# pyannote/pyannote-video

Hardware: AMD Instinct MI355X
Metric: frames/sec end-to-end detect->embed->cluster, 1080p@25fps (higher is better)
Workload: dtype f32 (detector scores, embedder) / f64 (tracker, clustering) / u8 frames; an f16 screening pass with a proven error bound decides which windows the detector's exact f32 chain is evaluated for -- results identical to dense f32 scoring (`dense_scoring`)

## Files before the change

pyannote-video_amd/csrc/api.hip:

```cpp
#include "pvf_internal.h"
#include <algorithm>
#include <cmath>
#include <cstdlib>
#include <string>
#include <thread>

#define API_BEGIN try {
#define API_END                                                        \
    return 0;                                                          \
    }                                                                  \
    catch (const std::exception& e) { pvf_set_error(e.what()); return -1; } \
    catch (...) { pvf_set_error("unknown error"); return -2; }

#define ENTER(c, h)                                                \
    Ctx* c = pvf_ctx(h);                                           \
    std::lock_guard<std::recursive_mutex> _api_lock(c->api_mu);    \
    HIP_CHECK(hipSetDevice(c->device))
#define ENTER_DET(c, h)                                            \
    Ctx* c = pvf_ctx(h);                                           \
    std::lock_guard<std::recursive_mutex> _det_lock(c->det_mu);    \
    HIP_CHECK(hipSetDevice(c->device))
#define ENTER_BOTH(c, h)                                           \
    Ctx* c = pvf_ctx(h);                                           \
    std::lock_guard<std::recursive_mutex> _det_lock(c->det_mu);    \
// ... 618 lines not shown
    for (int i = 0; i < n; ++i) f[i] = c->frame(frames[i]);
    ert_run(c, f, boxes, n, pts);
    API_END
}

extern "C" int32_t pvf_debug_landmarks_shape(pvf_handle h, const pvf_handle* frames, const pvf_rect_i32* boxes, int32_t n, int32_t* pts, float* shape)
{
    API_BEGIN
    ENTER(c, h);
    PVF_REQUIRE(n >= 0 && ((frames && boxes && pts && shape) || n == 0), "pvf_debug_landmarks_shape: bad arguments");
    if (n == 0) return 0;
    std::vector<Frame> f(n);
    for (int i = 0; i < n; ++i) f[i] = c->frame(frames[i]);
    ert_run(c, f, boxes, n, pts, shape);
    API_END
}

static uint8_t* make_face_chips(Ctx* c, const pvf_handle* frames, const int32_t* pts, int n)
{
    const EmbedModel& e = c->emb;
    PVF_REQUIRE(e.loaded, "embedder not loaded");
    std::vector<ChipJob> jobs(n);
    for (int i = 0; i < n; ++i) {
        ChipDetails d;
        face_chip_details(e, pts + (size_t)i * 68 * 2, &d);
        jobs[i] = chip_plan(c->frame(frames[i]), d);
    }
    const size_t bytes = (size_t)n * e.chip_size * e.chip_size * 3;
    c->s_trk0.ensure(bytes);
    chip_extract_batch(c, jobs, c->s_trk0.as<uint8_t>());
    return c->s_trk0.as<uint8_t>();
}

extern "C" int32_t pvf_face_chips(pvf_handle h, const pvf_handle* frames, const int32_t* pts, int32_t n, uint8_t* chips)
{
    API_BEGIN
    ENTER(c, h);
    if (n == 0) return 0;
    uint8_t* d = make_face_chips(c, frames, pts, n);
    HIP_CHECK(hipMemcpyAsync(chips, d, (size_t)n * 150 * 150 * 3, hipMemcpyDeviceToHost, c->stream));
    HIP_CHECK(hipStreamSynchronize(c->stream));
    API_END
}

extern "C" int32_t pvf_embed(pvf_handle h, const pvf_handle* frames, const int32_t* pts, int32_t n, float* out)
{
    API_BEGIN
    ENTER(c, h);
    if (n == 0) return 0;
    const int CH = 4096;
    for (int i0 = 0; i0 < n; i0 += CH) {
        const int m = std::min(CH, n - i0);
        uint8_t* d = make_face_chips(c, frames + i0, pts + (size_t)i0 * 136, m);
        resnet_forward(c, d, m, out + (size_t)i0 * 128);
    }
    API_END
}

extern "C" int32_t pvf_landmarks_embed(pvf_handle h, const pvf_handle* frames, const pvf_rect_i32* boxes, int32_t n, int32_t* pts, float* out)
{
    API_BEGIN
    ENTER(c, h);
    PVF_REQUIRE(n >= 0, "pvf_landmarks_embed: bad arguments");
    if (n == 0) return 0;
    PVF_REQUIRE(frames && boxes && pts && out, "pvf_landmarks_embed: bad arguments");
    {
        std::vector<Frame> f(n);
        for (int i = 0; i < n; ++i) f[i] = c->frame(frames[i]);
        ert_run(c, f, boxes, n, pts);
    }
    const int CH = 4096;
    for (int i0 = 0; i0 < n; i0 += CH) {
        const int m = std::min(CH, n - i0);
        uint8_t* d = make_face_chips(c, frames + i0, pts + (size_t)i0 * 136, m);
        resnet_forward(c, d, m, out + (size_t)i0 * 128);
    }
    API_END
}

extern "C" int32_t pvf_embed_chips(pvf_handle h, const uint8_t* chips, int32_t n, float* out)
{
    API_BEGIN
    ENTER(c, h);
    if (n == 0) return 0;
    const size_t bytes = (size_t)n * 150 * 150 * 3;
    c->s_trk0.ensure(bytes);
    HIP_CHECK(hipMemcpyAsync(c->s_trk0.p, chips, bytes, hipMemcpyHostToDevice, c->stream));
    resnet_forward(c, c->s_trk0.as<uint8_t>(), n, out);
    API_END
}

extern "C" int32_t pvf_jitter_plan(int32_t J, uint64_t seed, double* out)
{
    API_BEGIN
    jitter_check_count("pvf_jitter_plan", J);
    PVF_REQUIRE(out || J == 0, "pvf_jitter_plan: bad arguments");
    jitter_plan_rows(J, seed, out);
    API_END
}

static int32_t debug_jitter_chips(const char* who, pvf_handle h, const uint8_t* chips, int32_t n, int32_t J, uint64_t seed, uint8_t* out, bool via_transform)
{
    API_BEGIN
    ENTER(c, h);
    jitter_check_count(who, J);
    PVF_REQUIRE(n >= 0 && J >= 1 && ((chips && (out || via_transform)) || n == 0), std::string(who) + ": bad arguments");
    if (n == 0) return 0;
// ... 20 lines not shown
}

static int32_t jitter_entry_check(const char* who, int32_t n, int32_t J, bool pointers)
{
    API_BEGIN
    jitter_check_count(who, J);
    PVF_REQUIRE(n >= 0 && (pointers || n == 0), std::string(who) + ": bad arguments");
    API_END
}

extern "C" int32_t pvf_embed_jitter(pvf_handle h, const pvf_handle* frames, const int32_t* pts, int32_t n, int32_t J, uint64_t seed, float* out)
{
    if (jitter_entry_check("pvf_embed_jitter", n, J, frames && pts && out)) return -1;
    if (J <= 1) return pvf_embed(h, frames, pts, n, out);
    API_BEGIN
    ENTER(c, h);
    const int CH = 4096;
    for (int i0 = 0; i0 < n; i0 += CH) {
        const int m = std::min(CH, n - i0);
        uint8_t* d = make_face_chips(c, frames + i0, pts + (size_t)i0 * 136, m);
        jitter_embed_dev(c, d, m, J, seed, out + (size_t)i0 * 128);
    }
    API_END
}

extern "C" int32_t pvf_landmarks_embed_jitter(pvf_handle h, const pvf_handle* frames, const pvf_rect_i32* boxes, int32_t n, int32_t J, uint64_t seed,
                                              int32_t* pts, float* out)
{
    if (jitter_entry_check("pvf_landmarks_embed_jitter", n, J, frames && boxes && pts && out)) return -1;
    if (J <= 1) return pvf_landmarks_embed(h, frames, boxes, n, pts, out);
    API_BEGIN
    ENTER(c, h);
    if (n == 0) return 0;
    {
        std::vector<Frame> f(n);
        for (int i = 0; i < n; ++i) f[i] = c->frame(frames[i]);
        ert_run(c, f, boxes, n, pts);
    }
    const int CH = 4096;
    for (int i0 = 0; i0 < n; i0 += CH) {
        const int m = std::min(CH, n - i0);
        uint8_t* d = make_face_chips(c, frames + i0, pts + (size_t)i0 * 136, m);
        jitter_embed_dev(c, d, m, J, seed, out + (size_t)i0 * 128);
    }
    API_END
}

extern "C" int32_t pvf_embed_chips_jitter(pvf_handle h, const uint8_t* chips, int32_t n, int32_t J, uint64_t seed, float* out)
{
    if (jitter_entry_check("pvf_embed_chips_jitter", n, J, chips && out)) return -1;
    if (J <= 1) return pvf_embed_chips(h, chips, n, out);
    API_BEGIN
    ENTER(c, h);
    if (n == 0) return 0;
    const size_t bytes = (size_t)n * 150 * 150 * 3;
    c->s_trk0.ensure(bytes);
    HIP_CHECK(hipMemcpyAsync(c->s_trk0.p, chips, bytes, hipMemcpyHostToDevice, c->stream));
    jitter_embed_dev(c, c->s_trk0.as<uint8_t>(), n, J, seed, out);
    API_END
}

extern "C" int32_t pvf_debug_extract_chip(pvf_handle h, pvf_handle frame, const double rect[4], double cs, double sn, int32_t rows,
                                          int32_t cols, uint8_t* out)
{
    API_BEGIN
    ENTER(c, h);
    ChipDetails d{rect[0], rect[1], rect[2], rect[3], cs, sn, rows, cols};
    std::vector<ChipJob> jobs{chip_plan(c->frame(frame), d)};
    const size_t bytes = (size_t)rows * cols * 3;
    c->s_trk0.ensure(bytes);
    chip_extract_batch(c, jobs, c->s_trk0.as<uint8_t>());
    HIP_CHECK(hipMemcpyAsync(out, c->s_trk0.p, bytes, hipMemcpyDeviceToHost, c->stream));
    HIP_CHECK(hipStreamSynchronize(c->stream));
    API_END
}
// ... 415 lines not shown
```

pyannote-video_amd/csrc/chip.hip:

```cpp
#include "pvf_internal.h"
#include <algorithm>
#include <cmath>

static void pyr_down2_dims(int ih, int iw, int* oh, int* ow)
{
    if (ih <= 8 || iw <= 8) { *oh = 0; *ow = 0; return; }
    *oh = (ih - 3) / 2; *ow = (iw - 3) / 2;
}

ChipJob chip_plan(const Frame& f, const ChipDetails& d) { return chip_plan_geom(f.d, f.h, f.w, d); }

struct DevPyrJob { const uint8_t* src; int stride_w, x0, y0; uint8_t* dst; int dh, dw; };

#define PD_TW 32
#define PD_TH 8
__global__ void __launch_bounds__(256) pyr_down2_k(const DevPyrJob* __restrict__ jobs)
{
    __shared__ uint16_t hs[2 * PD_TH + 3][PD_TW][4];
    const DevPyrJob j = jobs[blockIdx.z];
    const int c0 = blockIdx.x * PD_TW, r0 = blockIdx.y * PD_TH;
    if (j.dst == nullptr || r0 >= j.dh || c0 >= j.dw) return;
    const int tid = threadIdx.x;
    const int rows_in = min(2 * PD_TH + 3, 2 * (j.dh - r0) + 3);
    for (int idx = tid; idx < (2 * PD_TH + 3) * PD_TW; idx += 256) {
        const int sr = idx / PD_TW, oc = idx % PD_TW;
        if (sr >= rows_in || c0 + oc >= j.dw) continue;
        const uint8_t* p = j.src + ((size_t)(j.y0 + 2 * r0 + sr) * j.stride_w + (j.x0 + 2 * (c0 + oc))) * 3;
        const uint32_t d0 = *reinterpret_cast<const uint32_t*>(p), d1 = *reinterpret_cast<const uint32_t*>(p + 4);
        const uint32_t d2 = *reinterpret_cast<const uint32_t*>(p + 8), d3 = *reinterpret_cast<const uint32_t*>(p + 11);
        const uint32_t h0 = (d0 & 0xffu) + 4 * (d0 >> 24) + 6 * ((d1 >> 16) & 0xffu) + 4 * ((d2 >> 8) & 0xffu) + ((d3 >> 8) & 0xffu);
        const uint32_t h1 = ((d0 >> 8) & 0xffu) + 4 * (d1 & 0xffu) + 6 * (d1 >> 24) + 4 * ((d2 >> 16) & 0xffu) + ((d3 >> 16) & 0xffu);
        const uint32_t h2 = ((d0 >> 16) & 0xffu) + 4 * ((d1 >> 8) & 0xffu) + 6 * (d2 & 0xffu) + 4 * (d2 >> 24) + (d3 >> 24);
        *reinterpret_cast<uint2*>(&hs[sr][oc][0]) = make_uint2(h0 | (h1 << 16), h2);
    }
    __syncthreads();
    const int c = c0 + (tid & (PD_TW - 1)), rl = tid >> 5, r = r0 + rl;
    if (r >= j.dh || c >= j.dw) return;
    const int oc = tid & (PD_TW - 1);
    uint32_t acc[3];
#pragma unroll
    for (int k = 0; k < 3; ++k)
        acc[k] = hs[2 * rl][oc][k] + 4u * hs[2 * rl + 1][oc][k] + 6u * hs[2 * rl + 2][oc][k] + 4u * hs[2 * rl + 3][oc][k] + hs[2 * rl + 4][oc][k];
    uint8_t* o = j.dst + ((size_t)r * j.dw + c) * 3;
    o[0] = (uint8_t)(acc[0] / 256); o[1] = (uint8_t)(acc[1] / 256); o[2] = (uint8_t)(acc[2] / 256);
}

__global__ void __launch_bounds__(256) transform_k(const DevXfJob* __restrict__ jobs, uint8_t* __restrict__ out, int rows, int cols)
{
    const DevXfJob j = jobs[blockIdx.z];
    const int c = blockIdx.x * blockDim.x + threadIdx.x;
    const int r = blockIdx.y;
    if (c >= cols) return;
    uint8_t* o = out + ((size_t)blockIdx.z * rows * cols + (size_t)r * cols + c) * 3;
    if (j.src == nullptr) { o[0] = 0; o[1] = 0; o[2] = 0; return; }
    const double px = j.m[0] * c + j.m[1] * r + j.b[0];
    const double py = j.m[2] * c + j.m[3] * r + j.b[1];
    const double fx = floor(px), fy = floor(py);
    if (!(fx >= 0 && fy >= 0 && fx + 1 < j.sw && fy + 1 < j.sh)) { o[0] = 0; o[1] = 0; o[2] = 0; return; }
    const int left = (int)fx, top = (int)fy;
    const double lr = px - left, tb = py - top;
    const uint8_t* ptl = j.src + ((size_t)(j.y0 + top) * j.stride_w + (j.x0 + left)) * 3;
    const uint8_t* pbl = ptl + (size_t)j.stride_w * 3;
    const uint32_t t0 = *reinterpret_cast<const uint32_t*>(ptl), t1 = *reinterpret_cast<const uint32_t*>(ptl + 2);
    const uint32_t b0 = *reinterpret_cast<const uint32_t*>(pbl), b1 = *reinterpret_cast<const uint32_t*>(pbl + 2);
    const uint32_t tl3[3] = {t0 & 0xffu, (t0 >> 8) & 0xffu, (t0 >> 16) & 0xffu}, tr3[3] = {t0 >> 24, (t1 >> 16) & 0xffu, t1 >> 24};
    const uint32_t bl3[3] = {b0 & 0xffu, (b0 >> 8) & 0xffu, (b0 >> 16) & 0xffu}, br3[3] = {b0 >> 24, (b1 >> 16) & 0xffu, b1 >> 24};
#pragma unroll
    for (int k = 0; k < 3; ++k) {
        const double tl = tl3[k], tr = tr3[k], bl = bl3[k], br = br3[k];
        const double v = (1 - tb) * ((1 - lr) * tl + lr * tr) + tb * ((1 - lr) * bl + lr * br);
        o[k] = (uint8_t)v;
    }
}

void transform_launch(Ctx* c, const DevXfJob* d_jobs, int n, int rows, int cols, uint8_t* d_out)
{
    hipLaunchKernelGGL(transform_k, dim3((cols + 63) / 64, rows, n), dim3(64), 0, c->stream, d_jobs, d_out, rows, cols);
}

void transform_batch(Ctx* c, const std::vector<ChipJob>& jobs, uint8_t* d_out)
{
    const int n = (int)jobs.size();
    if (n == 0) return;
    const int rows = jobs[0].rows, cols = jobs[0].cols;
    std::vector<DevXfJob> xf(n);
    for (int i = 0; i < n; ++i) {
        const ChipJob& j = jobs[i];
        DevXfJob& x = xf[i];
        x.src = j.img; x.stride_w = j.w; x.x0 = 0; x.y0 = 0; x.sw = j.w; x.sh = j.h;
        memcpy(x.m, j.m, sizeof x.m); memcpy(x.b, j.b, sizeof x.b);
    }
    c->s_chip.ensure(n * sizeof(DevXfJob));
    void* hb = c->stage.take(n * sizeof(DevXfJob));
    memcpy(hb, xf.data(), n * sizeof(DevXfJob));
    HIP_CHECK(hipMemcpyAsync(c->s_chip.p, hb, n * sizeof(DevXfJob), hipMemcpyHostToDevice, c->stream));
    c->stage.sent(c->stream);
    ProfScope ps(c, "chip");
    hipLaunchKernelGGL(transform_k, dim3((cols + 63) / 64, rows, n), dim3(64), 0, c->stream, c->s_chip.as<DevXfJob>(), d_out, rows, cols);
}

void chip_extract_batch(Ctx* c, const std::vector<ChipJob>& jobs, uint8_t* d_out)
{
    const int n = (int)jobs.size();
    if (n == 0) return;
    const int rows = jobs[0].rows, cols = jobs[0].cols;
    int max_levels = 0;
    for (auto& j : jobs) if (!j.empty) max_levels = std::max(max_levels, j.levels);
    std::vector<std::vector<DevPyrJob>> pj(max_levels, std::vector<DevPyrJob>(n));
    std::vector<DevXfJob> xf(n);
    size_t arena = 0;
    std::vector<size_t> offs;
    struct Slot { int job, level; size_t off; int h, w; };
    std::vector<Slot> slots;
    for (int i = 0; i < n; ++i) {
        const ChipJob& j = jobs[i];
        int ch = j.sh, cw = j.sw;
        for (int l = 0; l < j.levels && !j.empty; ++l) {
            int nh, nw;
            pyr_down2_dims(ch, cw, &nh, &nw);
            slots.push_back({i, l, arena, nh, nw});
            arena += ((size_t)std::max(nh, 0) * std::max(nw, 0) * 3 + 63) / 64 * 64;
            ch = nh; cw = nw;
        }
    }
    c->s_chip_pyr.ensure(arena + 64);
    uint8_t* base = c->s_chip_pyr.as<uint8_t>();
    for (int l = 0; l < max_levels; ++l)
        for (int i = 0; i < n; ++i) pj[l][i] = DevPyrJob{nullptr, 0, 0, 0, nullptr, 0, 0};
    std::vector<int> max_h(max_levels, 0), max_w(max_levels, 0);
    for (int i = 0; i < n; ++i) {
        const ChipJob& j = jobs[i];
// ... 9 lines not shown
        for (const Slot& s : slots) {
            const ChipJob& j = jobs[s.job];
            DevPyrJob& p = pj[s.level][s.job];
            if (s.level == 0) { p.src = j.img; p.stride_w = j.w; p.x0 = j.bx0; p.y0 = j.by0; }
            else { p.src = prev_ptr[s.job]; p.stride_w = prev_w[s.job]; p.x0 = 0; p.y0 = 0; }
            p.dst = (s.h > 0 && s.w > 0) ? base + s.off : nullptr;
            p.dh = s.h; p.dw = s.w;
            max_h[s.level] = std::max(max_h[s.level], s.h);
            max_w[s.level] = std::max(max_w[s.level], s.w);
            prev_ptr[s.job] = base + s.off; prev_h[s.job] = s.h; prev_w[s.job] = s.w;
            if (s.level == j.levels - 1) {
                DevXfJob& x = xf[s.job];
                if (s.h > 0 && s.w > 0) { x.src = base + s.off; x.stride_w = s.w; x.x0 = 0; x.y0 = 0; x.sw = s.w; x.sh = s.h; }
                else x.src = nullptr;
            }
        }
    }
    ScratchLayout lay;
    const auto sPyr = lay.take<DevPyrJob>((size_t)max_levels * n, 16); const auto sXf = lay.take<DevXfJob>(n, 16);
    const size_t used = lay.bytes();
    lay.pad(64);
    c->s_chip.ensure(lay.bytes());
    uint8_t* hb = reinterpret_cast<uint8_t*>(c->stage.take(lay.bytes()));
    for (int l = 0; l < max_levels; ++l) memcpy(hb + sPyr.off + (size_t)l * n * sizeof(DevPyrJob), pj[l].data(), n * sizeof(DevPyrJob));
    memcpy(hb + sXf.off, xf.data(), sXf.bytes());
    HIP_CHECK(hipMemcpyAsync(c->s_chip.p, hb, used, hipMemcpyHostToDevice, c->stream));
    c->stage.sent(c->stream);
    ProfScope ps(c, "chip");
    for (int l = 0; l < max_levels; ++l) {
        if (max_h[l] <= 0 || max_w[l] <= 0) continue;
        hipLaunchKernelGGL(pyr_down2_k, dim3((max_w[l] + PD_TW - 1) / PD_TW, (max_h[l] + PD_TH - 1) / PD_TH, n), dim3(256), 0, c->stream,
                           sPyr.in(c->s_chip) + (size_t)l * n);
    }
    hipLaunchKernelGGL(transform_k, dim3((cols + 63) / 64, rows, n), dim3(64), 0, c->stream, sXf.in(c->s_chip), d_out, rows, cols);
}
```

pyannote-video_amd/csrc/ert.hip:

```cpp
#include "pvf_internal.h"

struct ErtJob { const uint8_t* img; int h, w; int rect[4]; };

__device__ __forceinline__ int32_t sat_i32(double v) { return (int32_t)fmin(fmax(v, -2147483648.0), 2147483647.0); }

__global__ void __launch_bounds__(256) ert_k(const ErtJob* __restrict__ jobs, int n_cascades, int n_trees, int n_parts, int n_pix, int depth,
                                             const float* __restrict__ initial, const int32_t* __restrict__ anchor,
                                             const float* __restrict__ deltas, const int32_t* __restrict__ idx1,
                                             const int32_t* __restrict__ idx2, const float* __restrict__ thresh,
                                             const float* __restrict__ leaves, int32_t* __restrict__ pts,
                                             float* __restrict__ shape)
{
    extern __shared__ __attribute__((aligned(16))) float smem[];
    const int P2 = 2 * n_parts;
    float* cur = smem;
    float* pix = cur + ((P2 + 3) & ~3);
    int* leaf = reinterpret_cast<int*>(pix + ((n_pix + 3) & ~3));
    __shared__ float M[4];
    const ErtJob job = jobs[blockIdx.x];
    const int tid = threadIdx.x;
    const int n_split = (1 << depth) - 1, n_leaf = 1 << depth;
    const double sx = (double)job.rect[2] - (double)job.rect[0], sy = (double)job.rect[3] - (double)job.rect[1];
    const double ox = job.rect[0], oy = job.rect[1];
    for (int k = tid; k < P2; k += blockDim.x) cur[k] = initial[k];
    for (int it = 0; it < n_cascades; ++it) {
        __syncthreads();
        if (tid == 0) {
            double mfx = 0, mfy = 0, mtx = 0, mty = 0;
            for (int i = 0; i < n_parts; ++i) { mfx += initial[2 * i]; mfy += initial[2 * i + 1]; mtx += cur[2 * i]; mty += cur[2 * i + 1]; }
            mfx /= n_parts; mfy /= n_parts; mtx /= n_parts; mty /= n_parts;
            double a = 0, b = 0, s = 0;
            for (int i = 0; i < n_parts; ++i) {
                const double fx = initial[2 * i] - mfx, fy = initial[2 * i + 1] - mfy;
                const double tx = cur[2 * i] - mtx, ty = cur[2 * i + 1] - mty;
                a += fx * tx + fy * ty;
                b += fx * ty - fy * tx;
                s += fx * fx + fy * fy;
            }
            const double ca = a / s, cb = b / s;
            M[0] = (float)ca; M[1] = (float)(-cb); M[2] = (float)cb; M[3] = (float)ca;
        }
        __syncthreads();
        const int32_t* an = anchor + (size_t)it * n_pix;
        const float* dl = deltas + (size_t)it * n_pix * 2;
        for (int i = tid; i < n_pix; i += blockDim.x) {
            const float dx = dl[2 * i], dy = dl[2 * i + 1];
            const int ai = an[i];
            const float u = (M[0] * dx + M[1] * dy) + cur[2 * ai];
            const float v = (M[2] * dx + M[3] * dy) + cur[2 * ai + 1];
            const double X = (double)u * sx + ox, Y = (double)v * sy + oy;
            const long px = (long)floor(X + 0.5), py = (long)floor(Y + 0.5);
            float val = 0.0f;
            if (px >= 0 && py >= 0 && px < job.w && py < job.h) {
                const uint8_t* p = job.img + ((size_t)py * job.w + px) * 3;
                val = (float)(((unsigned)p[0] + p[1] + p[2]) / 3);
            }
            pix[i] = val;
        }
        __syncthreads();
        for (int t = tid; t < n_trees; t += blockDim.x) {
            const size_t sb = ((size_t)it * n_trees + t) * n_split;
            int i = 0;
            while (i < n_split) {
                if (pix[idx1[sb + i]] - pix[idx2[sb + i]] > thresh[sb + i]) i = 2 * i + 1;
                else i = 2 * i + 2;
            }
            leaf[t] = i - n_split;
        }
        __syncthreads();
        for (int k = tid; k < P2; k += blockDim.x) {
            float acc = cur[k];
            const float* lb = leaves + (size_t)it * n_trees * n_leaf * P2 + k;
            int t = 0;
            for (; t + 20 <= n_trees; t += 20) {
                float v[20];
#pragma unroll
                for (int j = 0; j < 20; ++j) v[j] = lb[((size_t)(t + j) * n_leaf + leaf[t + j]) * P2];
#pragma unroll
                for (int j = 0; j < 20; ++j) acc = acc + v[j];
            }
            for (; t < n_trees; ++t) acc = acc + lb[((size_t)t * n_leaf + leaf[t]) * P2];
            cur[k] = acc;
        }
    }
    __syncthreads();
    if (shape)
        for (int k = tid; k < P2; k += blockDim.x) shape[(size_t)blockIdx.x * P2 + k] = cur[k];
    for (int i = tid; i < n_parts; i += blockDim.x) {
        const double X = (double)cur[2 * i] * sx + ox, Y = (double)cur[2 * i + 1] * sy + oy;
        pts[((size_t)blockIdx.x * n_parts + i) * 2] = sat_i32(floor(X + 0.5));
        pts[((size_t)blockIdx.x * n_parts + i) * 2 + 1] = sat_i32(floor(Y + 0.5));
    }
}

void ert_run(Ctx* c, const std::vector<Frame>& frames, const pvf_rect_i32* boxes, int n, int32_t* pts, float* shape)
{
    const ShapeModel& s = c->shape;
    PVF_REQUIRE(s.loaded, "shape predictor not loaded");
    if (n == 0) return;
    std::vector<ErtJob> jobs(n);
    for (int i = 0; i < n; ++i) {
        jobs[i].img = frames[i].d; jobs[i].h = frames[i].h; jobs[i].w = frames[i].w;
        jobs[i].rect[0] = boxes[i].left; jobs[i].rect[1] = boxes[i].top; jobs[i].rect[2] = boxes[i].right; jobs[i].rect[3] = boxes[i].bottom;
    }
    ScratchLayout lay;
    const auto sJobs = lay.take<ErtJob>(n, 64); const auto sPts = lay.take<int32_t>((size_t)n * s.n_parts * 2, 64);
    const auto sShape = lay.take<float>(shape ? (size_t)n * s.n_parts * 2 : 0, 64);
    lay.pad(64);
    c->s_misc.ensure(lay.bytes());
    ErtJob* d_jobs = sJobs.in(c->s_misc); int32_t* d_pts = sPts.in(c->s_misc);
    float* d_shape = shape ? sShape.in(c->s_misc) : nullptr;
    HIP_CHECK(hipMemcpyAsync(d_jobs, jobs.data(), sJobs.bytes(), hipMemcpyHostToDevice, c->stream));
    const size_t lds = (size_t)(((2 * s.n_parts + 3) & ~3) + ((s.n_pix + 3) & ~3)) * 4 + (size_t)s.n_trees * 4;
    {
        ProfScope ps(c, "ert");
        hipLaunchKernelGGL(ert_k, dim3(n), dim3(256), lds, c->stream, d_jobs, s.n_cascades, s.n_trees,
                           s.n_parts, s.n_pix, s.depth, s.d_initial, s.d_anchor, s.d_deltas, s.d_idx1, s.d_idx2, s.d_thresh, s.d_leaves,
                           d_pts, d_shape);
    }
    HIP_CHECK(hipGetLastError());
    HIP_CHECK(hipMemcpyAsync(pts, d_pts, sPts.bytes(), hipMemcpyDeviceToHost, c->stream));
    if (shape) HIP_CHECK(hipMemcpyAsync(shape, d_shape, sShape.bytes(), hipMemcpyDeviceToHost, c->stream));
    HIP_CHECK(hipStreamSynchronize(c->stream));
}
```

pyannote-video_amd/csrc/pvf_internal.h:

```cpp
#pragma once
#include <hip/hip_runtime.h>
#include <cstdint>
#include <cstdio>
#include <cstring>
#include <deque>
#include <map>
#include <atomic>
#include <memory>
#include <mutex>
#include <stdexcept>
#include <string>
#include <unordered_map>
#include <vector>
#include "../../include/pvface.h"
#include "scratch_layout.h"
#include "chip_plan.h"
#include "group_blocks.h"

#define PVF_FHOG_STRIDE 32

struct CandOverflow : PvfError { int needed; explicit CandOverflow(int n) : PvfError("detector: candidate buffer overflow"), needed(n) {} };
struct ScreenRetry : PvfError { ScreenRetry() : PvfError("detector: screening pass gave up") {} };

#define HIP_CHECK(expr)                                                                              \
    do {                                                                                             \
        hipError_t _e = (expr);                                                                      \
        if (_e != hipSuccess) {                                                                      \
            char _b[512];                                                                            \
            snprintf(_b, sizeof _b, "%s failed: %s (%s:%d)", #expr, hipGetErrorString(_e), __FILE__, __LINE__); \
            throw PvfError(_b);                                                                      \
        }                                                                                            \
    } while (0)

#define PVF_REQUIRE(cond, msg)                     \
    do {                                           \
        if (!(cond)) throw PvfError(std::string(msg)); \
    } while (0)

// ... 148 lines not shown
constexpr size_t TRK_B = TRK_A + (size_t)32 * 64 * 64 * 2;
constexpr size_t TRK_AS = TRK_B + (size_t)64 * 64;
constexpr size_t TRK_BS = TRK_AS + (size_t)512 * 32 * 2;
constexpr size_t TRK_POS = TRK_BS + 32;
constexpr size_t TRK_DOUBLES = TRK_POS + 4;
constexpr size_t TRKF_PLANE = (size_t)64 * 64;
constexpr size_t TRKF_A = 5 * TRKF_PLANE * sizeof(float);
constexpr size_t TRKF_BYTES = TRKF_A + TRKF_PLANE;
#define TRKF_SLOT(q) ((((q) & 511) << 3) | ((q) >> 9))

struct DevXfJob { const uint8_t* src; int stride_w, x0, y0, sw, sh; double m[4], b[2]; };

struct Ctx {
    int device = 0;
    hipStream_t stream = nullptr;
    hipStream_t det_stream = nullptr;
    DetectorModel det;
    ShapeModel shape;
    EmbedModel emb;
    TrackerTables ttab;
    std::unordered_map<uint64_t, Frame> frames;
    std::unordered_map<uint64_t, std::unique_ptr<Tracker>> trackers;
    std::vector<double*> tracker_pool;
    std::atomic<uint64_t> next_id{1};
    std::recursive_mutex api_mu;
    std::recursive_mutex det_mu;
    std::mutex frames_mu;
    std::mutex prof_mu;
    bool prof_on = false;
    std::map<std::string, ProfFamily> prof;
    std::vector<hipEvent_t> event_pool;
    DevBuf s_grad, s_pyr, s_hist, s_norm, s_feat, s_cand, s_misc, s_chip, s_chip_pyr, s_act0, s_act1, s_act2, s_trk0, s_trk1, s_trk2, s_trkfeat, s_clu0, s_clu1;
    HostBuf h_cand, h_misc;
    StageRing stage;
    DevBuf s_cand2[2], s_fptr[2];
    HostBuf h_cand2[2], h_fptr[2];
    hipEvent_t det_ev[2] = {nullptr, nullptr};
    int det_slot = 0;
    int det_cand_cap = 8192;
    bool det_screen = true, det_screen_suspended = false, screen_attr_set = false;
    int screen_list_cap = 1 << 20;
    DevBuf s_screen;
    int64_t screen_batches = 0, screen_listed = 0, screen_retries = 0;
    double screen_pipe_err = -1;
    bool screen_pipe_flushes_subnormals = false;
    bool emb_split = true, emb_probe_done = false;
    DevBuf s_emb_flags, s_emb_redo;
    DevBuf s_jit;
    bool jit_attr_set = false;
    int64_t emb_split_faces = 0, emb_reruns = 0;
    double emb_pipe_err = -1;
    int n_cu = 256;
    struct PoolBuf { uint8_t* p; hipEvent_t free_after; hipEvent_t free_after_det; };
    std::map<size_t, std::deque<PoolBuf>> frame_pool;
    size_t frame_pool_bytes = 0;
    void* ingest_rings = nullptr;
    void* render_state = nullptr;
    void* tube_state = nullptr;
    void* board_state = nullptr;
    struct MlPlanCache* ml_plans = nullptr;
    std::map<std::vector<int>, std::unique_ptr<DevBuf>> resize_tabs;
    const void* feat_ring_owner = nullptr;
    uint8_t* d_orient_lut = nullptr;
    uint8_t* d_wrap_lut = nullptr;
    DevBuf s_orb_set, s_orb_work;
    int orb_n = 0, orb_cap = 0;
// ... 70 lines not shown
void det_run_batch(Ctx* c, const std::vector<Frame>& frames, int upsample, double adjust,
                   std::vector<std::vector<RawDet>>& raw_sorted);
void det_run_many(Ctx* c, const std::vector<Frame>& frames, int batch, int upsample, double adjust,
                  std::vector<std::vector<RawDet>>& raw_sorted, bool nms = false);
void ml_plans_free(Ctx* c);
void ingest_free_all(Ctx* c);
struct ResizeTab { std::vector<int32_t> idx; std::vector<int16_t> coef; };
ResizeTab linear_table(int in, int out);
void render_free_all(Ctx* c);
void tube_free_all(Ctx* c);
void board_free_all(Ctx* c);
void det_nms(const DetectorModel& m, const std::vector<RawDet>& sorted, std::vector<RawDet>& out);
void det_pyramid_level(Ctx* c, const Frame& f, int upsample, int level, std::vector<uint8_t>* out, int* h, int* w);
void det_level_features(Ctx* c, const Frame& f, int upsample, int level, std::vector<float>* out, int* fh, int* fw);
void det_level_plan(Ctx* c, const Frame& f, int upsample, int level, int32_t out[8]);
void det_pyramid_batch(Ctx* c, const std::vector<Frame>& frames, int upsample);
void fhog_debug(Ctx* c, const uint8_t* himg, int h, int w, int cell, int pad_r, int pad_c, std::vector<float>& out, int* fh, int* fw);
void fhog_device(Ctx* c, const uint8_t* d_img, int n, int h, int w, int cell, int pad_r, int pad_c, float* d_feat,
                 DevBuf& hist, DevBuf& norm, size_t img_stride_in = 0);
void fhog1_compact(Ctx* c, const uint8_t* d_chips, int n, uint8_t* d_rec);
void fhog_scale_chips(Ctx* c, const uint8_t* d_chips, int n, float* d_feat);
void fhog_dims(int ih, int iw, int cell, int pad_r, int pad_c, int* fh, int* fw);
ChipJob chip_plan(const Frame& f, const ChipDetails& d);
void chip_extract_batch(Ctx* c, const std::vector<ChipJob>& jobs, uint8_t* d_out );
void transform_batch(Ctx* c, const std::vector<ChipJob>& jobs, uint8_t* d_out);
void transform_launch(Ctx* c, const DevXfJob* d_jobs, int n, int rows, int cols, uint8_t* d_out);
void jitter_check_count(const char* who, int J);
void jitter_plan_rows(int J, uint64_t seed, double* out );
int jitter_faces_per_round(int J);
uint8_t* jitter_scratch(Ctx* c, int faces, int J);
void jitter_chips_dev(Ctx* c, const uint8_t* d_chips, int n, int J, uint64_t seed, uint8_t* d_out, bool via_transform);
void jitter_embed_dev(Ctx* c, const uint8_t* d_chips, int n, int J, uint64_t seed, float* out);
void ert_run(Ctx* c, const std::vector<Frame>& frames, const pvf_rect_i32* boxes, int n, int32_t* pts, float* shape = nullptr);
void face_chip_details(const EmbedModel& m, const int32_t* pts68, ChipDetails* out);
void dlib_mean_face_shape(float* out );
void resnet_forward(Ctx* c, const uint8_t* d_chips, int n, float* h_out);
struct ChipSource { const uint8_t* host; const pvf_handle* frames; const int32_t* pts; };
const EmbedModel& faces_geometry();
void faces_make_chips(Ctx* c, const pvf_handle* frames, const int32_t* pts, int m, uint8_t* d_chips);
void faces_source_round(Ctx* c, const ChipSource& src, int i0, int m, uint8_t* d_chips);
void sheet_check(const std::string& w, int W, int H, uint32_t background, const pvf_prim* prims, int n_prims, const uint8_t* text,
                 int64_t text_bytes, const uint8_t* rgb);
void sheet_prims_launch(Ctx* c, const pvf_prim* d_prims, int n_prims, const uint8_t* d_text, int W, int H, uint8_t* d_rgb);
void conv_layer_upload(ConvLayer& L, const float* w, const float* bias, const float* gamma, const float* beta);
void conv_layer_free(ConvLayer& L);
#define EMB_STAGES 30
struct EmbedTap { int stage; float* h_out; int dims[3]; };
void resnet_debug_stage(Ctx* c, const uint8_t* d_chips, int n, bool split, EmbedTap* tap, int* h_flags);
void resnet_debug_conv(Ctx* c, const int32_t* geom, const float* in, const float* w, const float* bias, const float* gamma, const float* beta,
                       const float* skip, bool split, bool force_generic, float* out, int32_t* flags);
void resnet_debug_head(Ctx* c, const float* x, int n, int hw, float* out);
void dsst_start_many(Ctx* c, const std::vector<Tracker*>& t, const std::vector<Frame>& f, const double* boxes);
void dsst_clone_many(Ctx* c, const std::vector<Tracker*>& src, const std::vector<Tracker*>& dst);
double* tracker_state_alloc(Ctx* c);
void shot_dfd(Ctx* c, const std::vector<Frame>& frames, int ow, int oh, const float* tables22, double* dfd, uint8_t* gray_out, float* flow_out);
std::vector<int> orb_level_quota();
void orb_extract(Ctx* c, const std::vector<Frame>& frames, int ow, int oh, int cap, int32_t* counts, float* kp_out, uint8_t* desc_out);
void orb_match_counts(Ctx* c, const uint8_t* desc, const int32_t* nrows, int n_sets, int cap, const int32_t* pairs, int64_t n_pairs, int32_t* out);
void dsst_update_many(Ctx* c, const std::vector<Tracker*>& t, const std::vector<Frame>& f, double* psr, double* boxes_out, int mode = 0);
void overlap_matrix_host(const double* a, int na, const double* b, int nb, double ratio, double* out);
void munkres_host(const double* cost, int n, int32_t* row_to_col);
struct PairInput {
    const double* X = nullptr;
    const float* emb = nullptr; int64_t emb_stride = 0; int n_src = 0; const int32_t* order = nullptr; int decimals = -1; bool emb_on_device = false;
};
struct PairOutput { double* out = nullptr; bool on_device = false; bool compact = false; };
// ... 28 lines not shown
```

Before: 4770.

## Chunk ERT landmarks to overlap host chip planning; flatten transform kernel grid

Landmark regression now runs in chunks, each with its own D2H copy and event. The host computes chip geometry for each finished chunk while later chunks still run on the GPU, so planning overlaps GPU work instead of following it. The chip transform kernel uses a flat 1D grid of 256-thread blocks in place of per-row 64-thread blocks, and an optional per-cascade ERT kernel mode (off by default, enabled by env var) is added. The cost is extra events, pinned host buffers and more code paths.

```diff
diff --git a/pyannote-video_amd/csrc/api.hip b/pyannote-video_amd/csrc/api.hip
--- a/pyannote-video_amd/csrc/api.hip
+++ b/pyannote-video_amd/csrc/api.hip
@@ -674,6 +674,42 @@
     return c->s_trk0.as<uint8_t>();
 }
 
+static int extract_chunk()
+{
+    const char* e = getenv("PVF_EXTRACT_CHUNK");
+    const int v = e ? atoi(e) : 0;
+    return v > 0 ? v : 4096;
+}
+
+static std::vector<ChipJob> landmarks_and_chip_plans(Ctx* c, const pvf_handle* frames, const pvf_rect_i32* boxes, int n, int32_t* pts)
+{
+    const EmbedModel& e = c->emb;
+    PVF_REQUIRE(e.loaded, "embedder not loaded");
+    std::vector<Frame> f(n);
+    for (int i = 0; i < n; ++i) f[i] = c->frame(frames[i]);
+    std::vector<ChipJob> jobs(n);
+    const auto plan = [&](int i0, int m) {
+        for (int i = i0; i < i0 + m; ++i) {
+            ChipDetails d;
+            face_chip_details(e, pts + (size_t)i * 68 * 2, &d);
+            jobs[i] = chip_plan(f[i], d);
+        }
+    };
+    const int chunk = extract_chunk();
+    if (n <= chunk) { ert_run(c, f, boxes, n, pts); plan(0, n); }
+    else ert_run_chunked(c, f, boxes, n, chunk, pts, plan);
+    return jobs;
+}
+
+static uint8_t* planned_face_chips(Ctx* c, const std::vector<ChipJob>& jobs, int i0, int m)
+{
+    const EmbedModel& e = c->emb;
+    c->s_trk0.ensure((size_t)m * e.chip_size * e.chip_size * 3);
+    if (i0 == 0 && m == (int)jobs.size()) chip_extract_batch(c, jobs, c->s_trk0.as<uint8_t>());
+    else chip_extract_batch(c, std::vector<ChipJob>(jobs.begin() + i0, jobs.begin() + i0 + m), c->s_trk0.as<uint8_t>());
+    return c->s_trk0.as<uint8_t>();
+}
+
 extern "C" int32_t pvf_face_chips(pvf_handle h, const pvf_handle* frames, const int32_t* pts, int32_t n, uint8_t* chips)
 {
     API_BEGIN
@@ -706,15 +742,11 @@
     PVF_REQUIRE(n >= 0, "pvf_landmarks_embed: bad arguments");
     if (n == 0) return 0;
     PVF_REQUIRE(frames && boxes && pts && out, "pvf_landmarks_embed: bad arguments");
-    {
-        std::vector<Frame> f(n);
-        for (int i = 0; i < n; ++i) f[i] = c->frame(frames[i]);
-        ert_run(c, f, boxes, n, pts);
-    }
+    const std::vector<ChipJob> jobs = landmarks_and_chip_plans(c, frames, boxes, n, pts);
     const int CH = 4096;
     for (int i0 = 0; i0 < n; i0 += CH) {
         const int m = std::min(CH, n - i0);
-        uint8_t* d = make_face_chips(c, frames + i0, pts + (size_t)i0 * 136, m);
+        uint8_t* d = planned_face_chips(c, jobs, i0, m);
         resnet_forward(c, d, m, out + (size_t)i0 * 128);
     }
     API_END
@@ -801,15 +833,11 @@
     API_BEGIN
     ENTER(c, h);
     if (n == 0) return 0;
-    {
-        std::vector<Frame> f(n);
-        for (int i = 0; i < n; ++i) f[i] = c->frame(frames[i]);
-        ert_run(c, f, boxes, n, pts);
-    }
+    const std::vector<ChipJob> jobs = landmarks_and_chip_plans(c, frames, boxes, n, pts);
     const int CH = 4096;
     for (int i0 = 0; i0 < n; i0 += CH) {
         const int m = std::min(CH, n - i0);
-        uint8_t* d = make_face_chips(c, frames + i0, pts + (size_t)i0 * 136, m);
+        uint8_t* d = planned_face_chips(c, jobs, i0, m);
         jitter_embed_dev(c, d, m, J, seed, out + (size_t)i0 * 128);
     }
     API_END
diff --git a/pyannote-video_amd/csrc/chip.hip b/pyannote-video_amd/csrc/chip.hip
--- a/pyannote-video_amd/csrc/chip.hip
+++ b/pyannote-video_amd/csrc/chip.hip
@@ -45,12 +45,14 @@
     o[0] = (uint8_t)(acc[0] / 256); o[1] = (uint8_t)(acc[1] / 256); o[2] = (uint8_t)(acc[2] / 256);
 }
 
-__global__ void __launch_bounds__(256) transform_k(const DevXfJob* __restrict__ jobs, uint8_t* __restrict__ out, int rows, int cols)
+#define XF_BLOCK 256
+__global__ void __launch_bounds__(XF_BLOCK) transform_k(const DevXfJob* __restrict__ jobs, uint8_t* __restrict__ out, int rows, int cols)
 {
     const DevXfJob j = jobs[blockIdx.z];
-    const int c = blockIdx.x * blockDim.x + threadIdx.x;
-    const int r = blockIdx.y;
-    if (c >= cols) return;
+    const uint32_t p = blockIdx.x * (uint32_t)XF_BLOCK + threadIdx.x;
+    if (p >= (uint32_t)rows * (uint32_t)cols) return;
+    const int r = (int)(p / (uint32_t)cols);
+    const int c = (int)(p - (uint32_t)r * (uint32_t)cols);
     uint8_t* o = out + ((size_t)blockIdx.z * rows * cols + (size_t)r * cols + c) * 3;
     if (j.src == nullptr) { o[0] = 0; o[1] = 0; o[2] = 0; return; }
     const double px = j.m[0] * c + j.m[1] * r + j.b[0];
@@ -75,7 +77,9 @@
 
 void transform_launch(Ctx* c, const DevXfJob* d_jobs, int n, int rows, int cols, uint8_t* d_out)
 {
-    hipLaunchKernelGGL(transform_k, dim3((cols + 63) / 64, rows, n), dim3(64), 0, c->stream, d_jobs, d_out, rows, cols);
+    PVF_REQUIRE(rows >= 1 && cols >= 1 && (int64_t)rows * cols <= INT32_MAX - XF_BLOCK, "chip: rows x cols out of range");
+    hipLaunchKernelGGL(transform_k, dim3(((unsigned)(rows * cols) + XF_BLOCK - 1) / XF_BLOCK, 1, n), dim3(XF_BLOCK), 0, c->stream, d_jobs, d_out,
+                       rows, cols);
 }
 
 void transform_batch(Ctx* c, const std::vector<ChipJob>& jobs, uint8_t* d_out)
@@ -96,7 +100,7 @@
     HIP_CHECK(hipMemcpyAsync(c->s_chip.p, hb, n * sizeof(DevXfJob), hipMemcpyHostToDevice, c->stream));
     c->stage.sent(c->stream);
     ProfScope ps(c, "chip");
-    hipLaunchKernelGGL(transform_k, dim3((cols + 63) / 64, rows, n), dim3(64), 0, c->stream, c->s_chip.as<DevXfJob>(), d_out, rows, cols);
+    transform_launch(c, c->s_chip.as<DevXfJob>(), n, rows, cols, d_out);
 }
 
 void chip_extract_batch(Ctx* c, const std::vector<ChipJob>& jobs, uint8_t* d_out)
@@ -172,5 +176,5 @@
         hipLaunchKernelGGL(pyr_down2_k, dim3((max_w[l] + PD_TW - 1) / PD_TW, (max_h[l] + PD_TH - 1) / PD_TH, n), dim3(256), 0, c->stream,
                            sPyr.in(c->s_chip) + (size_t)l * n);
     }
-    hipLaunchKernelGGL(transform_k, dim3((cols + 63) / 64, rows, n), dim3(64), 0, c->stream, sXf.in(c->s_chip), d_out, rows, cols);
+    transform_launch(c, sXf.in(c->s_chip), n, rows, cols, d_out);
 }
diff --git a/pyannote-video_amd/csrc/ert.hip b/pyannote-video_amd/csrc/ert.hip
--- a/pyannote-video_amd/csrc/ert.hip
+++ b/pyannote-video_amd/csrc/ert.hip
@@ -3,6 +3,105 @@
 struct ErtJob { const uint8_t* img; int h, w; int rect[4]; };
 
 __device__ __forceinline__ int32_t sat_i32(double v) { return (int32_t)fmin(fmax(v, -2147483648.0), 2147483647.0); }
+
+struct ErtLds { float* cur; float* pix; int* leaf; };
+__device__ __forceinline__ ErtLds ert_lds(float* smem, int P2, int n_pix)
+{
+    ErtLds l;
+    l.cur = smem;
+    l.pix = l.cur + ((P2 + 3) & ~3);
+    l.leaf = reinterpret_cast<int*>(l.pix + ((n_pix + 3) & ~3));
+    return l;
+}
+
+__device__ __forceinline__ void ert_cascade(const ErtJob& job, int it, int n_trees, int n_parts, int n_pix, int depth, const ErtLds& l, float* M,
+                                            const float* __restrict__ initial, const int32_t* __restrict__ anchor,
+                                            const float* __restrict__ deltas, const int32_t* __restrict__ idx1,
+                                            const int32_t* __restrict__ idx2, const float* __restrict__ thresh,
+                                            const float* __restrict__ leaves)
+{
+    float* cur = l.cur; float* pix = l.pix; int* leaf = l.leaf;
+    const int P2 = 2 * n_parts;
+    const int tid = threadIdx.x;
+    const int n_split = (1 << depth) - 1, n_leaf = 1 << depth;
+    const double sx = (double)job.rect[2] - (double)job.rect[0], sy = (double)job.rect[3] - (double)job.rect[1];
+    const double ox = job.rect[0], oy = job.rect[1];
+    __syncthreads();
+    if (tid == 0) {
+        double mfx = 0, mfy = 0, mtx = 0, mty = 0;
+        for (int i = 0; i < n_parts; ++i) { mfx += initial[2 * i]; mfy += initial[2 * i + 1]; mtx += cur[2 * i]; mty += cur[2 * i + 1]; }
+        mfx /= n_parts; mfy /= n_parts; mtx /= n_parts; mty /= n_parts;
+        double a = 0, b = 0, s = 0;
+        for (int i = 0; i < n_parts; ++i) {
+            const double fx = initial[2 * i] - mfx, fy = initial[2 * i + 1] - mfy;
+            const double tx = cur[2 * i] - mtx, ty = cur[2 * i + 1] - mty;
+            a += fx * tx + fy * ty;
+            b += fx * ty - fy * tx;
+            s += fx * fx + fy * fy;
+        }
+        const double ca = a / s, cb = b / s;
+        M[0] = (float)ca; M[1] = (float)(-cb); M[2] = (float)cb; M[3] = (float)ca;
+    }
+    __syncthreads();
+    const int32_t* an = anchor + (size_t)it * n_pix;
+    const float* dl = deltas + (size_t)it * n_pix * 2;
+    for (int i = tid; i < n_pix; i += blockDim.x) {
+        const float dx = dl[2 * i], dy = dl[2 * i + 1];
+        const int ai = an[i];
+        const float u = (M[0] * dx + M[1] * dy) + cur[2 * ai];
+        const float v = (M[2] * dx + M[3] * dy) + cur[2 * ai + 1];
+        const double X = (double)u * sx + ox, Y = (double)v * sy + oy;
+        const long px = (long)floor(X + 0.5), py = (long)floor(Y + 0.5);
+        float val = 0.0f;
+        if (px >= 0 && py >= 0 && px < job.w && py < job.h) {
+            const uint8_t* p = job.img + ((size_t)py * job.w + px) * 3;
+            val = (float)(((unsigned)p[0] + p[1] + p[2]) / 3);
+        }
+        pix[i] = val;
+    }
+    __syncthreads();
+    for (int t = tid; t < n_trees; t += blockDim.x) {
+        const size_t sb = ((size_t)it * n_trees + t) * n_split;
+        int i = 0;
+        while (i < n_split) {
+            if (pix[idx1[sb + i]] - pix[idx2[sb + i]] > thresh[sb + i]) i = 2 * i + 1;
+            else i = 2 * i + 2;
+        }
+        leaf[t] = i - n_split;
+    }
+    __syncthreads();
+    for (int k = tid; k < P2; k += blockDim.x) {
+        float acc = cur[k];
+        const float* lb = leaves + (size_t)it * n_trees * n_leaf * P2 + k;
+        int t = 0;
+        for (; t + 20 <= n_trees; t += 20) {
+            float v[20];
+#pragma unroll
+            for (int j = 0; j < 20; ++j) v[j] = lb[((size_t)(t + j) * n_leaf + leaf[t + j]) * P2];
+#pragma unroll
+            for (int j = 0; j < 20; ++j) acc = acc + v[j];
+        }
+        for (; t < n_trees; ++t) acc = acc + lb[((size_t)t * n_leaf + leaf[t]) * P2];
+        cur[k] = acc;
+    }
+}
+
+__device__ __forceinline__ void ert_finish(const ErtJob& job, int n_parts, const float* cur, size_t face, int32_t* __restrict__ pts,
+                                           float* __restrict__ shape)
+{
+    const int P2 = 2 * n_parts;
+    const int tid = threadIdx.x;
+    const double sx = (double)job.rect[2] - (double)job.rect[0], sy = (double)job.rect[3] - (double)job.rect[1];
+    const double ox = job.rect[0], oy = job.rect[1];
+    __syncthreads();
+    if (shape)
+        for (int k = tid; k < P2; k += blockDim.x) shape[face * P2 + k] = cur[k];
+    for (int i = tid; i < n_parts; i += blockDim.x) {
+        const double X = (double)cur[2 * i] * sx + ox, Y = (double)cur[2 * i + 1] * sy + oy;
+        pts[(face * n_parts + i) * 2] = sat_i32(floor(X + 0.5));
+        pts[(face * n_parts + i) * 2 + 1] = sat_i32(floor(Y + 0.5));
+    }
+}
 
 __global__ void __launch_bounds__(256) ert_k(const ErtJob* __restrict__ jobs, int n_cascades, int n_trees, int n_parts, int n_pix, int depth,
                                              const float* __restrict__ initial, const int32_t* __restrict__ anchor,
@@ -13,113 +112,139 @@
 {
     extern __shared__ __attribute__((aligned(16))) float smem[];
     const int P2 = 2 * n_parts;
-    float* cur = smem;
-    float* pix = cur + ((P2 + 3) & ~3);
-    int* leaf = reinterpret_cast<int*>(pix + ((n_pix + 3) & ~3));
+    const ErtLds l = ert_lds(smem, P2, n_pix);
     __shared__ float M[4];
     const ErtJob job = jobs[blockIdx.x];
-    const int tid = threadIdx.x;
-    const int n_split = (1 << depth) - 1, n_leaf = 1 << depth;
-    const double sx = (double)job.rect[2] - (double)job.rect[0], sy = (double)job.rect[3] - (double)job.rect[1];
-    const double ox = job.rect[0], oy = job.rect[1];
-    for (int k = tid; k < P2; k += blockDim.x) cur[k] = initial[k];
-    for (int it = 0; it < n_cascades; ++it) {
-        __syncthreads();
-        if (tid == 0) {
-            double mfx = 0, mfy = 0, mtx = 0, mty = 0;
-            for (int i = 0; i < n_parts; ++i) { mfx += initial[2 * i]; mfy += initial[2 * i + 1]; mtx += cur[2 * i]; mty += cur[2 * i + 1]; }
-            mfx /= n_parts; mfy /= n_parts; mtx /= n_parts; mty /= n_parts;
-            double a = 0, b = 0, s = 0;
-            for (int i = 0; i < n_parts; ++i) {
-                const double fx = initial[2 * i] - mfx, fy = initial[2 * i + 1] - mfy;
-                const double tx = cur[2 * i] - mtx, ty = cur[2 * i + 1] - mty;
-                a += fx * tx + fy * ty;
-                b += fx * ty - fy * tx;
-                s += fx * fx + fy * fy;
-            }
-            const double ca = a / s, cb = b / s;
-            M[0] = (float)ca; M[1] = (float)(-cb); M[2] = (float)cb; M[3] = (float)ca;
-        }
-        __syncthreads();
-        const int32_t* an = anchor + (size_t)it * n_pix;
-        const float* dl = deltas + (size_t)it * n_pix * 2;
-        for (int i = tid; i < n_pix; i += blockDim.x) {
-            const float dx = dl[2 * i], dy = dl[2 * i + 1];
-            const int ai = an[i];
-            const float u = (M[0] * dx + M[1] * dy) + cur[2 * ai];
-            const float v = (M[2] * dx + M[3] * dy) + cur[2 * ai + 1];
-            const double X = (double)u * sx + ox, Y = (double)v * sy + oy;
-            const long px = (long)floor(X + 0.5), py = (long)floor(Y + 0.5);
-            float val = 0.0f;
-            if (px >= 0 && py >= 0 && px < job.w && py < job.h) {
-                const uint8_t* p = job.img + ((size_t)py * job.w + px) * 3;
-                val = (float)(((unsigned)p[0] + p[1] + p[2]) / 3);
-            }
-            pix[i] = val;
-        }
-        __syncthreads();
-        for (int t = tid; t < n_trees; t += blockDim.x) {
-            const size_t sb = ((size_t)it * n_trees + t) * n_split;
-            int i = 0;
-            while (i < n_split) {
-                if (pix[idx1[sb + i]] - pix[idx2[sb + i]] > thresh[sb + i]) i = 2 * i + 1;
-                else i = 2 * i + 2;
-            }
-            leaf[t] = i - n_split;
-        }
-        __syncthreads();
-        for (int k = tid; k < P2; k += blockDim.x) {
-            float acc = cur[k];
-            const float* lb = leaves + (size_t)it * n_trees * n_leaf * P2 + k;
-            int t = 0;
-            for (; t + 20 <= n_trees; t += 20) {
-                float v[20];
-#pragma unroll
-                for (int j = 0; j < 20; ++j) v[j] = lb[((size_t)(t + j) * n_leaf + leaf[t + j]) * P2];
-#pragma unroll
-                for (int j = 0; j < 20; ++j) acc = acc + v[j];
-            }
-            for (; t < n_trees; ++t) acc = acc + lb[((size_t)t * n_leaf + leaf[t]) * P2];
-            cur[k] = acc;
-        }
-    }
-    __syncthreads();
-    if (shape)
-        for (int k = tid; k < P2; k += blockDim.x) shape[(size_t)blockIdx.x * P2 + k] = cur[k];
-    for (int i = tid; i < n_parts; i += blockDim.x) {
-        const double X = (double)cur[2 * i] * sx + ox, Y = (double)cur[2 * i + 1] * sy + oy;
-        pts[((size_t)blockIdx.x * n_parts + i) * 2] = sat_i32(floor(X + 0.5));
-        pts[((size_t)blockIdx.x * n_parts + i) * 2 + 1] = sat_i32(floor(Y + 0.5));
-    }
-}
-
-void ert_run(Ctx* c, const std::vector<Frame>& frames, const pvf_rect_i32* boxes, int n, int32_t* pts, float* shape)
-{
-    const ShapeModel& s = c->shape;
-    PVF_REQUIRE(s.loaded, "shape predictor not loaded");
-    if (n == 0) return;
-    std::vector<ErtJob> jobs(n);
+    for (int k = threadIdx.x; k < P2; k += blockDim.x) l.cur[k] = initial[k];
+    for (int it = 0; it < n_cascades; ++it)
+        ert_cascade(job, it, n_trees, n_parts, n_pix, depth, l, M, initial, anchor, deltas, idx1, idx2, thresh, leaves);
+    ert_finish(job, n_parts, l.cur, blockIdx.x, pts, shape);
+}
+
+__global__ void __launch_bounds__(256) ert_cascade_k(const ErtJob* __restrict__ jobs, int it, int last, int n_trees, int n_parts, int n_pix, int depth,
+                                                     const float* __restrict__ initial, const int32_t* __restrict__ anchor,
+                                                     const float* __restrict__ deltas, const int32_t* __restrict__ idx1,
+                                                     const int32_t* __restrict__ idx2, const float* __restrict__ thresh,
+                                                     const float* __restrict__ leaves, float* __restrict__ state,
+                                                     int32_t* __restrict__ pts, float* __restrict__ shape)
+{
+    extern __shared__ __attribute__((aligned(16))) float smem[];
+    const int P2 = 2 * n_parts;
+    const ErtLds l = ert_lds(smem, P2, n_pix);
+    __shared__ float M[4];
+    const ErtJob job = jobs[blockIdx.x];
+    const float* from = it == 0 ? initial : state + (size_t)blockIdx.x * P2;
+    for (int k = threadIdx.x; k < P2; k += blockDim.x) l.cur[k] = from[k];
+    ert_cascade(job, it, n_trees, n_parts, n_pix, depth, l, M, initial, anchor, deltas, idx1, idx2, thresh, leaves);
+    if (last) { ert_finish(job, n_parts, l.cur, blockIdx.x, pts, shape); return; }
+    __syncthreads();
+    for (int k = threadIdx.x; k < P2; k += blockDim.x) state[(size_t)blockIdx.x * P2 + k] = l.cur[k];
+}
+
+static bool ert_cascade_major()
+{
+    const char* e = getenv("PVF_ERT_CASCADES");
+    return e && atoi(e) != 0;
+}
+
+struct ErtScratch { ErtJob* jobs; int32_t* pts; float* shape; float* state; bool cascades; };
+
+static ErtScratch ert_upload(Ctx* c, const std::vector<Frame>& frames, const pvf_rect_i32* boxes, int n, bool want_shape)
+{
+    const ShapeModel& s = c->shape;
+    ErtJob* jobs = reinterpret_cast<ErtJob*>(c->stage.take((size_t)n * sizeof(ErtJob)));
     for (int i = 0; i < n; ++i) {
         jobs[i].img = frames[i].d; jobs[i].h = frames[i].h; jobs[i].w = frames[i].w;
         jobs[i].rect[0] = boxes[i].left; jobs[i].rect[1] = boxes[i].top; jobs[i].rect[2] = boxes[i].right; jobs[i].rect[3] = boxes[i].bottom;
     }
+    const size_t P2 = (size_t)s.n_parts * 2;
     ScratchLayout lay;
-    const auto sJobs = lay.take<ErtJob>(n, 64); const auto sPts = lay.take<int32_t>((size_t)n * s.n_parts * 2, 64);
-    const auto sShape = lay.take<float>(shape ? (size_t)n * s.n_parts * 2 : 0, 64);
+    const auto sJobs = lay.take<ErtJob>(n, 64); const auto sPts = lay.take<int32_t>((size_t)n * P2, 64);
+    const auto sShape = lay.take<float>(want_shape ? (size_t)n * P2 : 0, 64);
+    const bool cascades = ert_cascade_major() && s.n_cascades >= 1;
+    const auto sState = lay.take<float>(cascades ? (size_t)n * P2 : 0, 64);
     lay.pad(64);
     c->s_misc.ensure(lay.bytes());
-    ErtJob* d_jobs = sJobs.in(c->s_misc); int32_t* d_pts = sPts.in(c->s_misc);
-    float* d_shape = shape ? sShape.in(c->s_misc) : nullptr;
-    HIP_CHECK(hipMemcpyAsync(d_jobs, jobs.data(), sJobs.bytes(), hipMemcpyHostToDevice, c->stream));
+    ErtScratch d{sJobs.in(c->s_misc), sPts.in(c->s_misc), want_shape ? sShape.in(c->s_misc) : nullptr, sState.in(c->s_misc), cascades};
+    HIP_CHECK(hipMemcpyAsync(d.jobs, jobs, sJobs.bytes(), hipMemcpyHostToDevice, c->stream));
+    c->stage.sent(c->stream);
+    return d;
+}
+
+static void ert_launch(Ctx* c, const ErtScratch& d, int i0, int m)
+{
+    const ShapeModel& s = c->shape;
+    const size_t P2 = (size_t)s.n_parts * 2;
     const size_t lds = (size_t)(((2 * s.n_parts + 3) & ~3) + ((s.n_pix + 3) & ~3)) * 4 + (size_t)s.n_trees * 4;
+    const ErtJob* jobs = d.jobs + i0;
+    int32_t* pts = d.pts + (size_t)i0 * P2;
+    float* shape = d.shape ? d.shape + (size_t)i0 * P2 : nullptr;
+    float* state = d.state + (size_t)i0 * P2;
     {
         ProfScope ps(c, "ert");
-        hipLaunchKernelGGL(ert_k, dim3(n), dim3(256), lds, c->stream, d_jobs, s.n_cascades, s.n_trees,
-                           s.n_parts, s.n_pix, s.depth, s.d_initial, s.d_anchor, s.d_deltas, s.d_idx1, s.d_idx2, s.d_thresh, s.d_leaves,
-                           d_pts, d_shape);
+        if (!d.cascades)
+            hipLaunchKernelGGL(ert_k, dim3(m), dim3(256), lds, c->stream, jobs, s.n_cascades, s.n_trees,
+                               s.n_parts, s.n_pix, s.depth, s.d_initial, s.d_anchor, s.d_deltas, s.d_idx1, s.d_idx2, s.d_thresh, s.d_leaves,
+                               pts, shape);
+        else
+            for (int it = 0; it < s.n_cascades; ++it)
+                hipLaunchKernelGGL(ert_cascade_k, dim3(m), dim3(256), lds, c->stream, jobs, it, it == s.n_cascades - 1 ? 1 : 0, s.n_trees,
+                                   s.n_parts, s.n_pix, s.depth, s.d_initial, s.d_anchor, s.d_deltas, s.d_idx1, s.d_idx2, s.d_thresh, s.d_leaves,
+                                   state, pts, shape);
     }
     HIP_CHECK(hipGetLastError());
-    HIP_CHECK(hipMemcpyAsync(pts, d_pts, sPts.bytes(), hipMemcpyDeviceToHost, c->stream));
-    if (shape) HIP_CHECK(hipMemcpyAsync(shape, d_shape, sShape.bytes(), hipMemcpyDeviceToHost, c->stream));
+}
+
+void ert_run(Ctx* c, const std::vector<Frame>& frames, const pvf_rect_i32* boxes, int n, int32_t* pts, float* shape)
+{
+    const ShapeModel& s = c->shape;
+    PVF_REQUIRE(s.loaded, "shape predictor not loaded");
+    if (n == 0) return;
+    const ErtScratch d = ert_upload(c, frames, boxes, n, shape != nullptr);
+    ert_launch(c, d, 0, n);
+    const size_t P2 = (size_t)s.n_parts * 2;
+    HIP_CHECK(hipMemcpyAsync(pts, d.pts, (size_t)n * P2 * sizeof(int32_t), hipMemcpyDeviceToHost, c->stream));
+    if (shape) HIP_CHECK(hipMemcpyAsync(shape, d.shape, (size_t)n * P2 * sizeof(float), hipMemcpyDeviceToHost, c->stream));
     HIP_CHECK(hipStreamSynchronize(c->stream));
 }
+
+namespace {
+struct EventList {
+    std::vector<hipEvent_t> ev;
+    ~EventList() { for (hipEvent_t e : ev) (void)hipEventDestroy(e); }
+};
+}
+
+void ert_run_chunked(Ctx* c, const std::vector<Frame>& frames, const pvf_rect_i32* boxes, int n, int chunk, int32_t* pts,
+                     const std::function<void(int, int)>& on_chunk)
+{
+    const ShapeModel& s = c->shape;
+    PVF_REQUIRE(s.loaded, "shape predictor not loaded");
+    PVF_REQUIRE(chunk >= 1, "landmark chunk: at least one face");
+    if (n == 0) return;
+    const size_t P2 = (size_t)s.n_parts * 2;
+    const ErtScratch d = ert_upload(c, frames, boxes, n, false);
+    c->h_ert.ensure((size_t)n * P2 * sizeof(int32_t));
+    int32_t* h = c->h_ert.as<int32_t>();
+    EventList done;
+    for (int i0 = 0; i0 < n; i0 += chunk) {
+        const int m = std::min(chunk, n - i0);
+        ert_launch(c, d, i0, m);
+        HIP_CHECK(hipMemcpyAsync(h + (size_t)i0 * P2, d.pts + (size_t)i0 * P2, (size_t)m * P2 * sizeof(int32_t), hipMemcpyDeviceToHost, c->stream));
+        hipEvent_t e;
+        HIP_CHECK(hipEventCreateWithFlags(&e, hipEventDisableTiming));
+        done.ev.push_back(e);
+        HIP_CHECK(hipEventRecord(e, c->stream));
+    }
+    try {
+        for (int i0 = 0, k = 0; i0 < n; i0 += chunk, ++k) {
+            const int m = std::min(chunk, n - i0);
+            HIP_CHECK(hipEventSynchronize(done.ev[k]));
+            memcpy(pts + (size_t)i0 * P2, h + (size_t)i0 * P2, (size_t)m * P2 * sizeof(int32_t));
+            on_chunk(i0, m);
+        }
+    } catch (...) {
+        (void)hipStreamSynchronize(c->stream);
+        throw;
+    }
+}
diff --git a/pyannote-video_amd/csrc/pvf_internal.h b/pyannote-video_amd/csrc/pvf_internal.h
--- a/pyannote-video_amd/csrc/pvf_internal.h
+++ b/pyannote-video_amd/csrc/pvf_internal.h
@@ -4,6 +4,7 @@
 #include <cstdio>
 #include <cstring>
 #include <deque>
+#include <functional>
 #include <map>
 #include <atomic>
 #include <memory>
@@ -218,6 +219,7 @@
     std::vector<hipEvent_t> event_pool;
     DevBuf s_grad, s_pyr, s_hist, s_norm, s_feat, s_cand, s_misc, s_chip, s_chip_pyr, s_act0, s_act1, s_act2, s_trk0, s_trk1, s_trk2, s_trkfeat, s_clu0, s_clu1;
     HostBuf h_cand, h_misc;
+    HostBuf h_ert;
     StageRing stage;
     DevBuf s_cand2[2], s_fptr[2];
     HostBuf h_cand2[2], h_fptr[2];
@@ -354,6 +356,8 @@
 void jitter_chips_dev(Ctx* c, const uint8_t* d_chips, int n, int J, uint64_t seed, uint8_t* d_out, bool via_transform);
 void jitter_embed_dev(Ctx* c, const uint8_t* d_chips, int n, int J, uint64_t seed, float* out);
 void ert_run(Ctx* c, const std::vector<Frame>& frames, const pvf_rect_i32* boxes, int n, int32_t* pts, float* shape = nullptr);
+void ert_run_chunked(Ctx* c, const std::vector<Frame>& frames, const pvf_rect_i32* boxes, int n, int chunk, int32_t* pts,
+                     const std::function<void(int, int)>& on_chunk);
 void face_chip_details(const EmbedModel& m, const int32_t* pts68, ChipDetails* out);
 void dlib_mean_face_shape(float* out );
 void resnet_forward(Ctx* c, const uint8_t* d_chips, int n, float* h_out);
```

After: 4787, median of 2. Within noise of the previous version (+0.3%).
